# jermp/dint

Hardware: AMD Instinct MI355X
Metric: M ints/sec decoded (vroom single_packed_dint) (higher is better)
Workload: dtype u32

## Files before the change

dint_amd/csrc/hip/dint_kernels.hpp:

```cpp
#pragma once
#include <hip/hip_runtime.h>
#include <stdint.h>

#include "dint_hip.h"

namespace dint_dev {

#ifndef DINT_STORE_AUX
#define DINT_STORE_AUX 2
#endif
#ifndef DINT_BLOCK_THREADS
#define DINT_BLOCK_THREADS 1024
#endif
#ifndef DINT_FF_OPEN
#define DINT_FF_OPEN 4
#endif
#ifndef DINT_MAX_STRAGGLERS
#define DINT_MAX_STRAGGLERS 4096
#endif
#ifndef DINT_SLOT_BURST
#define DINT_SLOT_BURST 2
#endif
static_assert(DINT_SLOT_BURST == 1 || DINT_SLOT_BURST == 2, "DINT_SLOT_BURST: 1 or 2");
#ifndef DINT_SLOT_GLOBAL
#define DINT_SLOT_GLOBAL (DINT_SLOT_BURST == 2)
#endif
#ifndef DINT_SLOT_LATE
#define DINT_SLOT_LATE 0
#endif
#ifndef DINT_GATHER_AUX
#define DINT_GATHER_AUX 0
#endif

constexpr uint32_t kWave = 64;
constexpr uint32_t kBlockThreads = DINT_BLOCK_THREADS;
constexpr uint32_t kWavesPerBlock = kBlockThreads / kWave;
constexpr uint32_t kBlocksPerCU = 1;
constexpr uint32_t kLdsWords = 160 * 1024 / 4;
constexpr uint32_t kSPL = 4;
constexpr uint32_t kTileSlots = kWave * kSPL;
#ifndef DINT_GROUPS
#define DINT_GROUPS 2
#endif
constexpr uint32_t kGroups = DINT_GROUPS;
constexpr uint32_t kRounds = 8 / kGroups;
constexpr uint32_t kMaxCap = 2048;
constexpr uint32_t kFwWords = 2 * 64 + 4;
constexpr uint32_t kDeltaWords = kTileSlots + 4;
#ifndef DINT_STAGE_CELLS
#define DINT_STAGE_CELLS 176
#endif
constexpr uint32_t kStageWords = 4 * DINT_STAGE_CELLS;
#ifdef DINT_PROFILE
constexpr uint32_t kProfWords = 16;
#else
constexpr uint32_t kProfWords = 0;
#endif
constexpr uint32_t kScratchWords = kFwWords + kDeltaWords + kStageWords + kProfWords;
constexpr uint32_t kClassTableWords = 328 + 24;
constexpr uint32_t kDescWordAt = 328;
constexpr uint32_t kHotImageWords = kLdsWords - kClassTableWords - kWavesPerBlock * kScratchWords;
constexpr uint32_t kZeroHalves = 256;
constexpr uint32_t kMetaCold = 1u << 23;
constexpr uint32_t kMetaSlow = 1u << 22;
constexpr uint32_t kMetaOffMask = (1u << 20) - 2;
constexpr uint32_t kMetaPacked8 = 1u;
constexpr uint32_t kMetaException = 1u << 20;
constexpr uint32_t kQueueShards = 8;
constexpr uint32_t kQueueStride = 32;
constexpr uint32_t kChunkShards = 32;
constexpr uint32_t kChunkCounterLineAt = 1;
constexpr uint32_t kQueueLines = kQueueShards + 1 + kChunkShards;
constexpr uint32_t kClockWordAt = 16;
constexpr uint32_t kChunkDryWordAt = 24;
constexpr uint32_t kUnitDryWordAt = 25;
constexpr uint32_t kMaxUnitInts = 1u << 28;

#include "kernels/wave_basics.inc"
#include "kernels/tile.inc"
#include "kernels/segment.inc"
#include "kernels/bundles.inc"

}
#include "dint_query_kernels.hpp"
namespace dint_dev {

#include "kernels/index.inc"
#include "kernels/kernel_body.inc"
#include "kernels/query_pages.inc"

__global__ void debug_wave_scan_kernel(const uint32_t* in, uint32_t* out) {
    out[threadIdx.x] = wave_inclusive_sum(in[threadIdx.x]);
}

}
```

dint_amd/csrc/hip/kernels/bundles.inc:

```
__device__ __forceinline__ void decode_unit_single(const decode_args& a, const wave_ctx& c, uint64_t unit_index, prof_t& pf) {
    const dint_unit* up = a.units + unit_index;
    const uint64_t out_off = up->out_off;
    const uint32_t n = up->n;
    if (n == 0 || n > kMaxUnitInts || out_off > a.out_capacity || a.out_capacity - out_off < n || (a.only_full && n != 256)) return;
    const uint64_t in_off = uniform64(up->in_off);
    chain_io ch{};
    volatile uint8_t* const flag = a.unit_base ? a.gaps_left + unit_index : nullptr;
    if (flag && c.lane == 0) *flag = 0;
    const uint64_t end = decode_segment<16, kRounds, kGroups, 0>(a, c, a.dict.first, in_off, n, a.out + out_off, ch, pf, false, false,
                                                                 a.unit_base ? a.unit_base + unit_index : nullptr,
                                                                 a.unit_base ? a.gaps_left + unit_index : nullptr);
    if (a.end_off && c.lane == 0) a.end_off[unit_index] = end;
    if (flag && n <= 256) {
        uint32_t left = 0;
        if (c.lane == 0) left = *flag, *flag = 0;
        if (uniform(left) != 0) gaps_to_docids_here(a.out + out_off, n, uniform(a.unit_base[unit_index]), c.lane);
    }
}

constexpr uint32_t kBundleMaxInts = 256;
constexpr uint32_t kBundleMaxBytes = 504;

constexpr uint32_t kChunkUnits = 64;
__global__ __launch_bounds__(256) void bundle_schedule_kernel(const dint_unit* units, const uint32_t* spans, uint64_t n_units,
                                                              const uint8_t* enc, uint64_t enc_bytes, uint64_t out_capacity,
                                                              uint32_t only_full, uint32_t multi, uint32_t chunked, uint8_t* sched,
                                                              uint32_t* block_items, u32x4* urec, uint64_t* cbase) {
    __shared__ uint32_t lanes[256], pre[256];
    __shared__ uint32_t place[256];
    __shared__ uint8_t start[256];
    const uint32_t tid = threadIdx.x;
    const uint64_t i = uint64_t(blockIdx.x) * 256 + tid;
    uint32_t L = 0, sel = 0;
    uint64_t in = 0, out = 0;
    uint32_t n = 0;
    if (i < n_units) {
        in = units[i].in_off;
        out = units[i].out_off;
        n = units[i].n;
    }
    const uint64_t in0 = (uint64_t(uint32_t(__shfl(uint32_t(in >> 32), 0))) << 32) | uint32_t(__shfl(uint32_t(in), 0));
    const uint64_t out0 = (uint64_t(uint32_t(__shfl(uint32_t(out >> 32), 0))) << 32) | uint32_t(__shfl(uint32_t(out), 0));
    if (i < n_units) {
        const uint64_t nxt = spans ? in + spans[i] : (i + 1 < n_units ? units[i + 1].in_off : enc_bytes);
        if (n >= 1 && n <= kBundleMaxInts && (!only_full || n == 256) && nxt > in && nxt - in <= kBundleMaxBytes &&
            nxt <= enc_bytes && out <= out_capacity && out_capacity - out >= n && in >= in0 && nxt - in0 + 16 <= 0xFFFFFFFFull && out >= out0 &&
            out - out0 < (chunked ? (1ull << 28) : (1ull << 32))) {
            if (!multi) {
                const uint32_t l = uint32_t((nxt - in + 7) >> 3);
                if (l <= kWave - 1 && in + 8ull * l <= enc_bytes) L = l;
            } else {
                sel = enc[in];
                const uint32_t stride = sel >= 6 ? 4u : 8u;
                const uint32_t l = uint32_t((nxt - in - 1 + stride - 1) / stride);
                if (sel < 12 && l >= 1 && l <= kWave - 1 && in + 1 + uint64_t(stride) * l + 8 <= enc_bytes) L = l;
            }
        }
    }
    lanes[tid] = L | (n << 8);
    pre[tid] = (L != 0 && tid != 0 && i < n_units && out == units[i - 1].out_off + units[i - 1].n) ? 1u : 0u;
    __syncthreads();
    if (chunked) {
        start[tid] = L != 0 ? 0 : 1;
        place[tid] = 0;
    } else if ((tid & 63u) == 0) {
        uint32_t in_use = 0, ints = 0, prev_l = 0;
#pragma unroll 16
        for (uint32_t j = tid; j != tid + 64; ++j) {
            const uint32_t l = lanes[j] & 255u, m = lanes[j] >> 8;
            const bool cont = l != 0 && prev_l != 0 && pre[j] != 0 && in_use + l <= kWave && ints + m <= kMaxCap;
            start[j] = cont ? 0 : 1;
            in_use = cont ? in_use + l : l;
            ints = cont ? ints + m : m;
            prev_l = l;
        }
    }
    __syncthreads();
    uint32_t c = 0;
    if (start[tid] != 0 && i < n_units) {
        c = 1;
        if (L != 0 && !chunked)
            while (tid + c < 256 && ((tid + c) & 63u) != 0 && i + c < n_units && !start[tid + c]) ++c;
    }
    const bool alone = c == 1 && (L == 0 || !chunked) && !(chunked && only_full && n != 256);
    const bool item = alone || (!chunked && c > 1);
    const int n_items = __syncthreads_count(item);
    if (tid == 0) block_items[blockIdx.x] = uint32_t(n_items);
    if (i >= n_units) return;
    sched[i] = uint8_t(item ? c : 0);
    u32x4 r;
    r.x = uint32_t(in - in0);
    r.y = uint32_t(out - out0);
    r.z = ((n - 1u) & 255u) | (L << 8) | (sel << 14) | (c << 18);
    r.w = chunked ? place[tid] : 0u;
    urec[i] = r;
    if ((tid & 63u) == 0) {
        cbase[2 * (i >> 6)] = in0;
        cbase[2 * (i >> 6) + 1] = out0;
    }
}

__global__ __launch_bounds__(64) void bundle_pack_kernel(u32x4* urec, uint64_t n_units) {
    __shared__ uint32_t zs[64][65];
    constexpr uint32_t kOpen = DINT_FF_OPEN;
    const uint32_t tid = threadIdx.x;
    const uint64_t base = (uint64_t(blockIdx.x) * 64 + tid) * kChunkUnits;
    for (uint32_t j = 0; j != kChunkUnits; ++j) zs[tid][j] = base + j < n_units ? urec[base + j].z : 0u;
    uint32_t used[kOpen], mem[kOpen], id[kOpen], n_open = 0, next_id = 0;
#pragma unroll
    for (uint32_t k = 0; k != kOpen; ++k) used[k] = 0, mem[k] = 0, id[k] = 0;
    for (uint32_t j = 0; j != kChunkUnits; ++j) {
        const uint32_t z = zs[tid][j];
        const uint32_t l = (z >> 8) & 63u;
        uint32_t b = kOpen;
#pragma unroll
        for (uint32_t k = 0; k != kOpen; ++k)
            if (b == kOpen && k < n_open && used[k] + l <= kWave && mem[k] < 8) b = k;
        const bool fresh = b == kOpen;
        if (fresh) {
            b = n_open < kOpen ? n_open : 0u;
            if (n_open == kOpen) {
                uint32_t most = used[0];
#pragma unroll
                for (uint32_t k = 1; k != kOpen; ++k)
                    if (used[k] > most) most = used[k], b = k;
            }
        }
        uint32_t pl = 0;
#pragma unroll
        for (uint32_t k = 0; k != kOpen; ++k)
            if (k == b && l != 0) {
                if (fresh) id[k] = next_id, used[k] = 0, mem[k] = 0;
                pl = id[k] | (used[k] << 8) | (mem[k] << 16) | (mem[k] == 0 ? 1u << 31 : 0u);
                used[k] += l;
                mem[k] += 1;
            }
        if (fresh && l != 0) {
            next_id += 1;
            n_open += n_open < kOpen ? 1u : 0u;
        }
        zs[tid][j] = pl;
    }
    for (uint32_t j = 0; j != kChunkUnits; ++j) {
        const uint32_t pl = zs[tid][j];
        if (base + j < n_units && pl != 0) {
            u32x4 r = urec[base + j];
            r.z = (r.z & ~(127u << 18)) | ((pl >> 31) << 18);
            r.w = pl & 0x7FFFFFFFu;
            urec[base + j] = r;
        }
    }
}

__global__ __launch_bounds__(256) void split_units_kernel(const uint32_t* items, uint32_t n_items, const dint_unit* units, const uint8_t* enc,
                                                          uint64_t enc_bytes, uint64_t out_capacity, dict_view dv, u32x4* urec, uint64_t* cbase,
                                                          uint32_t* left_items, uint32_t* n_left) {
    const uint32_t j = blockIdx.x * 256 + threadIdx.x;
    if (j >= n_items) return;
    const dint_unit u = units[items[j]];
    const dint_unit u0 = units[items[j & ~31u]];
    const uint64_t in0 = u0.in_off, out0 = u0.out_off;
    if ((j & 31u) == 0) {
// ... 786 lines not shown
```

dint_amd/csrc/hip/kernels/kernel_body.inc:

```
struct query_pages {
    const dint_block_ref* blocks;
    const uint32_t* ids;
    const uint32_t* count;
    uint64_t bound;
    uint32_t retire;
    const uint32_t* page_query;
    const uint32_t* term_first;
    const uint32_t* term_blocks;
    const uint32_t* block_max;
    uint32_t* target;
    uint32_t* needed;
    uint32_t* rank;
    uint32_t* touched;
    uint32_t* n_touched;
    uint32_t hash_mask;
};
template <bool MULTI>
__device__ __forceinline__ void decode_query_page(const decode_args& a, const wave_ctx& c, const query_pages& qp, uint64_t page, prof_t& pf);

template <bool ALL = true>
__device__ __forceinline__ decode_args own_scalars(const decode_args& k) {
    decode_args a = k;
    asm volatile("" : "+s"(a.dict.tables), "+s"(a.dict.lds_image), "+s"(a.dict.descs), "+s"(a.dict.tables_bytes),
                 "+s"(a.dict.heads_base), "+s"(a.dict.tails_base), "+s"(a.dict.goff_base), "+s"(a.dict.gtable_base), "+s"(a.dict.hot_words),
                 "+s"(a.dict.first.meta_base), "+s"(a.dict.first.hot_base), "+s"(a.dict.first.hot_k));
    asm volatile("" : "+s"(a.enc), "+s"(a.enc_bytes), "+s"(a.units), "+s"(a.n_units), "+s"(a.out),
                 "+s"(a.out_capacity), "+s"(a.end_off), "+s"(a.queue), "+s"(a.n_shards), "+s"(a.only_full));
    if (ALL) asm volatile("" : "+s"(a.sched), "+s"(a.items), "+s"(a.item_cnt), "+s"(a.n_items), "+s"(a.urec), "+s"(a.cbase), "+s"(a.chunk_queue), "+s"(a.spans),
                 "+s"(a.plus_one), "+s"(a.unit_base), "+s"(a.gaps_left));
    return a;
}

template <bool MULTI, bool INDEX, bool QUERY = false, bool BUNDLES_ONLY = false>
__device__ __forceinline__ void decode_kernel_body(const decode_args& kernarg, const query_pages* qp = nullptr,
                                                   const round_tail* tail = nullptr, const tails_args* short_blocks = nullptr,
                                                   uint32_t karg_at = 0) {
    decode_args a_ = own_scalars<(MULTI || INDEX || QUERY)>(kernarg);
    if (!INDEX) {
        a_.unit_base = nullptr;
        a_.gaps_left = nullptr;
        a_.plus_one = 0;
        a_.only_full = 0;
    }
    const decode_args a = a_;
    const uint64_t clock0 = __builtin_amdgcn_s_memtime();
    extern __shared__ __attribute__((aligned(16))) uint32_t lds[];
    uint64_t q_work = 0;
    if (QUERY) {
        q_work = qp->bound;
        if (qp->count) q_work = uniform(*qp->count) < q_work ? uniform(*qp->count) : q_work;
    }
    const bool q_idle = QUERY && uint64_t(blockIdx.x) * kWavesPerBlock >= q_work;
    if (!q_idle) {
    if (!QUERY) {
        for (uint32_t i = threadIdx.x; 4 * i < a.dict.hot_words; i += kBlockThreads)
            reinterpret_cast<u32x4*>(lds)[i] = reinterpret_cast<const u32x4*>(a.dict.lds_image)[i];
    } else {
        constexpr uint32_t kSteps = (kHotImageWords / 4 + kBlockThreads - 1) / kBlockThreads;
        u32x4 part[kSteps];
#pragma unroll
        for (uint32_t k = 0; k != kSteps; ++k) {
            const uint32_t i = threadIdx.x + k * kBlockThreads;
            if (4 * i < a.dict.hot_words) part[k] = reinterpret_cast<const u32x4*>(a.dict.lds_image)[i];
        }
#pragma unroll
        for (uint32_t k = 0; k != kSteps; ++k) {
            const uint32_t i = threadIdx.x + k * kBlockThreads;
            if (4 * i < a.dict.hot_words) reinterpret_cast<u32x4*>(lds)[i] = part[k];
        }
    }
    uint16_t* const cls = reinterpret_cast<uint16_t*>(lds + a.dict.hot_words);
    build_class_table(cls);
    uint32_t* const descs = lds + a.dict.hot_words + kDescWordAt;
    if (threadIdx.x < 24) descs[threadIdx.x] = MULTI ? reinterpret_cast<const uint32_t*>(a.dict.descs)[threadIdx.x] : 0u;
    const uint32_t lane = lane_id();
    const uint32_t wave = uniform(threadIdx.x / kWave);
    uint32_t* const scratch = lds + a.dict.hot_words + kClassTableWords + wave * kScratchWords;
    for (uint32_t i = lane; i < kFwWords; i += kWave) scratch[i] = 0;
    __syncthreads();
    wave_ctx c;
    c.lds = lds;
    c.cls = cls;
    c.descs = descs;
    c.scratch = scratch;
    c.lane = lane;
    c.rs_dict = __builtin_amdgcn_make_buffer_rsrc(const_cast<uint8_t*>(a.dict.tables), 0, int(a.dict.tables_bytes), 0x00020000);
    c.heads_base = a.dict.heads_base;
    c.tails_base = a.dict.tails_base;
    c.goff_base = a.dict.goff_base;
    c.gtable_base = a.dict.gtable_base;
    const uint32_t shard = blockIdx.x % a.n_shards;
    const uint64_t n_work = QUERY ? q_work : a.sched ? uint64_t(uniform(*a.n_items)) : a.n_units;
    const uint64_t per_shard = (n_work + a.n_shards - 1) / a.n_shards;
    uint32_t cur = shard;
    auto ask = [&]() -> uint32_t {
        uint32_t j = 0;
        if (lane == 0) j = __hip_atomic_fetch_add(a.queue + cur * kQueueStride, 1u, __ATOMIC_RELAXED, __HIP_MEMORY_SCOPE_AGENT);
        return j;
    };
    auto take = [&](uint32_t ticket) -> uint64_t {
        uint32_t j = uniform(ticket);
        for (;;) {
            const uint64_t first = per_shard * cur;
            const uint64_t size = first >= n_work ? 0 : (n_work - first < per_shard ? n_work - first : per_shard);
            if (j < size) return first + j;
            const uint32_t next = next_open_counter(a.chunk_queue + kUnitDryWordAt, a.n_shards, cur, lane);
            if (next == ~0u) return ~0ull;
            cur = next;
            j = uniform(ask());
        }
    };
    prof_t pf;
#ifdef DINT_PROFILE
    prof_begin(pf, scratch + kScratchWords - kProfWords, lane);
#endif
    if (INDEX && !QUERY && short_blocks) {
        if (short_blocks->zero_next != nullptr && blockIdx.x == gridDim.x - 1)
            for (uint32_t i = threadIdx.x; i < short_blocks->zero_words; i += kBlockThreads) short_blocks->zero_next[i] = 0;
        SECTION(pf, 5, "short_blocks");
        tails_phase(a.enc, a.enc_bytes, *short_blocks, uint32_t(scratch - lds), lane);
        SECTION(pf, 0, "outside");
    }
    if (QUERY) {
        const uint64_t stride = uint64_t(gridDim.x) * kWavesPerBlock;
        for (uint64_t page = uint64_t(blockIdx.x) * kWavesPerBlock + wave; page < n_work; page += stride) decode_query_page<MULTI>(a, c, *qp, page, pf);
    }
    uint64_t w = BUNDLES_ONLY || QUERY ? ~0ull : take(ask());
    while (!BUNDLES_ONLY && !QUERY && w != ~0ull) {
        SECTION(pf, 14, "draw");
        uint32_t ticket = ask();
        const uint64_t uu = uniform64(!QUERY && a.sched ? uint64_t(a.items[w]) : w);
        if (QUERY) {
            decode_query_page<MULTI>(a, c, *qp, uu, pf);
        } else if (MULTI) {
            decode_unit_multi(a, c, uu, pf);
        } else {
            const uint32_t cc = uniform(a.sched ? uint32_t(a.item_cnt[w]) : 1u);
            if (__builtin_expect(cc > 1, 0)) decode_bundle_listed<false>(a, c, uu, cc, pf);
            else decode_unit_single(a, c, uu, pf);
        }
        asm volatile("" : "+v"(ticket));
        w = take(ticket);
    }
    if ((MULTI || (INDEX && a.only_full)) && !QUERY && a.sched && a.urec) {
        decode_bundle_chunks<MULTI, (MULTI && !INDEX && BUNDLES_ONLY)>(a, c, pf);
    }
#ifdef DINT_PROFILE
    prof_end(pf);
#endif
    }
    if (blockIdx.x == 0 && threadIdx.x == 0 && (a.urec || !a.sched))
    {
#if defined(__HIP_DEVICE_COMPILE__)
        typedef __attribute__((address_space(4))) const uint8_t constant_u8;
        constant_u8* kp = (constant_u8*)__builtin_amdgcn_kernarg_segment_ptr();
        asm volatile("" : "+s"(kp));
        uint64_t* const clk = *(uint64_t* __attribute__((address_space(4))) const*)(kp + karg_at + offsetof(decode_args, clock));
        *clk = __builtin_amdgcn_s_memtime() - clock0;
#else
        (void)clock0, (void)karg_at;
#endif
    }
    if (QUERY) {
        if (!tail->done) return;
        __shared__ uint32_t last;
        if (gridDim.x != 1) __threadfence();
        __syncthreads();
        if (gridDim.x != 1) {
            if (threadIdx.x == 0) last = atomicAdd(tail->done, 1u) == gridDim.x - 1 ? 1u : 0u;
            __syncthreads();
            if (!last) return;
            __threadfence();
        }
        and_round_tail(*tail);
    }
}

#ifndef DINT_MIN_WAVES
#define DINT_MIN_WAVES 1
#endif
__global__ __launch_bounds__(kBlockThreads, DINT_MIN_WAVES) void decode_single_kernel(decode_args a) {
    decode_kernel_body<false, false>(a);
}
__global__ __launch_bounds__(kBlockThreads, DINT_MIN_WAVES) void decode_multi_kernel(decode_args a) {
    decode_kernel_body<true, false>(a);
}
__global__ __launch_bounds__(kBlockThreads, DINT_MIN_WAVES) __attribute__((amdgpu_num_vgpr(126))) void decode_multi_bundles_kernel(decode_args a) {
    decode_kernel_body<true, false, false, true>(a);
}
__global__ __launch_bounds__(kBlockThreads, DINT_MIN_WAVES) void decode_single_index_kernel(decode_args a, tails_args t) {
    decode_kernel_body<false, true>(a, nullptr, nullptr, &t);
}
__global__ __launch_bounds__(kBlockThreads, DINT_MIN_WAVES) void decode_multi_index_kernel(decode_args a, tails_args t) {
    decode_kernel_body<true, true>(a, nullptr, nullptr, &t);
}
__global__ __launch_bounds__(kBlockThreads, DINT_MIN_WAVES) void decode_single_index_bundles_kernel(decode_args a, tails_args t) {
    decode_kernel_body<false, true, false, true>(a, nullptr, nullptr, &t);
}
__global__ __launch_bounds__(kBlockThreads, DINT_MIN_WAVES) void decode_multi_index_bundles_kernel(decode_args a, tails_args t) {
    decode_kernel_body<true, true, false, true>(a, nullptr, nullptr, &t);
}
__global__ __launch_bounds__(kBlockThreads, DINT_MIN_WAVES) void decode_single_index_pair_kernel(decode_args a, decode_args b, tails_args t) {
    decode_kernel_body<false, true, false, true>(a, nullptr, nullptr, &t);
    __syncthreads();
    decode_kernel_body<false, true, false, true>(b, nullptr, nullptr, nullptr, uint32_t(sizeof(decode_args)));
}
__global__ __launch_bounds__(kBlockThreads, DINT_MIN_WAVES) void decode_multi_index_pair_kernel(decode_args a, decode_args b, tails_args t) {
    decode_kernel_body<true, true, false, true>(a, nullptr, nullptr, &t);
    __syncthreads();
    decode_kernel_body<true, true, false, true>(b, nullptr, nullptr, nullptr, uint32_t(sizeof(decode_args)));
}
```

dint_amd/csrc/hip/kernels/segment.inc:

```
template <int W, uint32_t ROUNDS, uint32_t GROUPS, int CHAINED_T>
__device__ __forceinline__ uint64_t decode_segment(const decode_args& a, const wave_ctx& c, const dict_desc& dd, uint64_t in_off,
                                                   uint32_t n, uint32_t* const out, chain_io& ch, prof_t& pf,
                                                   bool narrow_rt = false, bool chained_rt = false,
                                                   const uint32_t* block_base = nullptr, uint8_t* gaps_left = nullptr) {
    SECTION(pf, 11, "segment_prologue");
    docid_bases gb;
    if (block_base != nullptr) gb.v = *block_base;
    const bool narrow = W == 0 ? narrow_rt : W == 8;
    const bool CHAINED = CHAINED_T < 0 ? chained_rt : CHAINED_T != 0;
    const uint32_t kSlotBytes = narrow ? 1u : 2u;
    const uint32_t kTileBytes = kTileSlots * kSlotBytes;
    const uint16_t* const rows = c.cls + (!narrow ? 0 : kRows16);
    const uint32_t lane = c.lane;
    const uint32_t hot_k = dd.hot_k;
    uint32_t* const out_u = reinterpret_cast<uint32_t*>(uniform64(reinterpret_cast<uint64_t>(out)));
    const __amdgpu_buffer_rsrc_t rs_out = __builtin_amdgcn_make_buffer_rsrc(out_u, 0, int(uniform(n) * 4), 0x00020000);
    uint8_t* const lds_rw = reinterpret_cast<uint8_t*>(const_cast<uint32_t*>(c.lds));
    const uint32_t stage_byte0 = uint32_t(reinterpret_cast<const uint8_t*>(stage_of(c.scratch)) - lds_rw);

    constexpr bool kPaired = DINT_SLOT_BURST == 2 && W == 16 && CHAINED_T == 0;
    constexpr bool kGlobalSlots = DINT_SLOT_GLOBAL != 0 && W == 16 && CHAINED_T == 0;
    constexpr bool kLateSlots = DINT_SLOT_LATE != 0 && W == 16 && CHAINED_T == 0;
    const uint64_t in_off_u = uniform64(in_off);
    uint64_t slot_byte = in_off_u;
    uint32_t room = 0;
    if (kPaired && in_off_u <= a.enc_bytes) room = uniform(a.enc_bytes - in_off_u < 0xFFFFFFFFull ? uint32_t(a.enc_bytes - in_off_u) : 0xFFFFFFFFu);
    tile_regs cur;
    uint64_t nxt_raw;
    meta_regs mr;
    head_regs hr;
    uint64_t raw1, raw2 = 0;
    if (CHAINED) {
        unpack_slots(narrow, chain_tile(narrow, ch.data, 0, lane), cur);
        raw1 = chain_tile(narrow, ch.data, 1, lane);
        slot_byte += kTileBytes;
    } else {
        uint64_t raw0 = load_lane_slots<kGlobalSlots>(narrow, a.enc, slot_byte, lane, a.enc_bytes);
        slot_byte += kTileBytes;
        raw1 = load_lane_slots<kGlobalSlots>(narrow, a.enc, slot_byte, lane, a.enc_bytes);
        slot_byte += kTileBytes;
        raw2 = load_lane_slots<kGlobalSlots>(narrow, a.enc, slot_byte, lane, a.enc_bytes);
        asm volatile("" : "+v"(raw0), "+v"(raw1), "+v"(raw2));
        unpack_slots(narrow, raw0, cur);
    }
    ch.valid = false;
    struct tile_class {
        uint32_t row;
        uint32_t carry_out;
        bool special;
        bool tile_exc;
    };
    auto classify = [&](const tile_regs& tr, uint32_t carry_in) -> tile_class {
        tile_class k{kPlainRow, 0u, false, false};
        uint32_t smin = tr.s[0];
#pragma unroll
        for (uint32_t j = 1; j != kSPL; ++j) smin = smin < tr.s[j] ? smin : tr.s[j];
        k.special = __builtin_expect(__ballot(smin < 2) != 0 || carry_in != 0, 0);
        if (k.special) {
            uint32_t lo = 0;
#pragma unroll
            for (uint32_t j = kSPL; j-- != 0;) lo = 3 * lo + (2u - (tr.s[j] < 2 ? tr.s[j] : 2u));
            uint32_t st_in = lane == 0 ? carry_in : 0u;
            uint32_t row;
            for (;;) {
                row = rows[st_in * 81 + lo];
                uint32_t prev = from_lane_below((row >> 8) & 7u);
                if (lane == 0) prev = carry_in;
                if (__ballot(prev != st_in) == 0) break;
                st_in = prev;
            }
            k.row = row;
            k.carry_out = readlane((row >> 8) & 7u, 63);
            k.tile_exc = __ballot((row & 0xF0u) != 0) != 0;
        }
        return k;
    };
    tile_class kc = classify(cur, 0u);
    request_metas(c, dd.hot_base, hot_k, dd.meta_base, cur, mr, hr, kc.row & 15u);
    asm volatile("" : "+v"(raw1), "+v"(raw2));
    nxt_raw = raw1;

    uint32_t produced = 0;
    uint64_t tile_base = in_off_u;
    uint32_t end_slot = 0;
    MARK("loop_top");

    while (produced < n) {
        uint64_t raw3;
        if (!kPaired && !kLateSlots) {
            slot_byte += kTileBytes;
            raw3 = load_lane_slots<kGlobalSlots>(narrow, a.enc, slot_byte, lane, a.enc_bytes);
        }

        SECTION(pf, 1, "1_classify");
        take_metas(hot_k, mr, hr, cur);
        if (!kPaired && kLateSlots) {
            slot_byte += kTileBytes;
            raw3 = load_lane_slots<kGlobalSlots>(narrow, a.enc, slot_byte, lane, a.enc_bytes);
        }
        if (kPaired) {
            if (uint32_t(slot_byte - tile_base) == kTileBytes) {
                const uint64_t pair_byte = slot_byte + kTileBytes;
                slot_byte += 2 * kTileBytes;
                if (uint32_t(slot_byte - in_off_u) + kTileBytes <= room) {
                    raw2 = load_lane_slots<kGlobalSlots, true>(narrow, a.enc, pair_byte, lane, a.enc_bytes);
                    raw3 = load_lane_slots<kGlobalSlots, true>(narrow, a.enc, slot_byte, lane, a.enc_bytes);
                } else {
                    raw2 = load_lane_slots<kGlobalSlots>(narrow, a.enc, pair_byte, lane, a.enc_bytes);
                    raw3 = load_lane_slots<kGlobalSlots>(narrow, a.enc, slot_byte, lane, a.enc_bytes);
                }
            } else {
                asm volatile("" : "=v"(raw3));
            }
        }
        const bool special = kc.special;
        const uint32_t row = kc.row;
        const uint32_t carry_out = kc.carry_out;
        const bool tile_exc = kc.tile_exc;

        SECTION(pf, 2, "2_sizes");
        tile_slots t;
        uint32_t lv1[kSPL] = {1u, 1u, 1u, 1u};
        if (special) {
#pragma unroll
            for (uint32_t k = 0; k != kSPL; ++k) {
                cur.m[k] &= uint32_t(__builtin_amdgcn_sbfe(~row, k, 1));
                lv1[k] = __builtin_amdgcn_ubfe(~row, k, 1);
            }
        }
        const bool tile_slow_dict = __ballot(((cur.m[0] | cur.m[1] | cur.m[2] | cur.m[3]) & kMetaSlow) != 0) != 0;
        uint32_t e[kSPL];
#pragma unroll
        for (uint32_t k = 0; k != kSPL; ++k) {
            e[k] = cur.m[k] >> 24;
            t.need[k] = __builtin_amdgcn_ubfe(cur.m[k], 20, 2);
            t.src2[k] = cur.m[k] & kMetaOffMask;
        }
        bool wide[kSPL] = {false, false, false, false};
        if (tile_exc) {
            uint32_t w32[kSPL];
            if (!narrow) {
                const uint32_t p01 = (cur.s[1] << 16) | cur.s[0], p23 = (cur.s[3] << 16) | cur.s[2];
                const uint32_t next0 = readlane(uint32_t(nxt_raw), 0);
                uint32_t nlo = from_lane_above(p01);
                if (lane == 63) nlo = next0;
                w32[0] = __builtin_amdgcn_alignbit(p23, p01, 16);
                w32[1] = p23;
                w32[2] = __builtin_amdgcn_alignbit(nlo, p23, 16);
                w32[3] = nlo;
            } else {
                const uint32_t b = cur.s[0] | (cur.s[1] << 8) | (cur.s[2] << 16) | (cur.s[3] << 24);
                const uint32_t next0 = readlane(uint32_t(nxt_raw), 0);
                uint32_t nlo = from_lane_above(b);
                if (lane == 63) nlo = next0;
                w32[0] = __builtin_amdgcn_alignbit(nlo, b, 8);
                w32[1] = __builtin_amdgcn_alignbit(nlo, b, 16);
                w32[2] = __builtin_amdgcn_alignbit(nlo, b, 24);
                w32[3] = nlo;
            }
#pragma unroll
            for (uint32_t k = 0; k != kSPL; ++k) {
                const uint32_t excM = uint32_t(__builtin_amdgcn_sbfe(row, 4 + k, 1));
                const uint32_t lit = w32[k] & ((0u - cur.s[k]) | 0xFFFFu) & excM;
                hr.q[k].y = (hr.q[k].y & ~excM) | lit;
                wide[k] = lit > 0xFFFFu;
            }
        }
        t.off[0] = 0;
        t.off[1] = e[0] + lv1[0];
        t.off[2] = t.off[1] + e[1] + lv1[1];
        t.off[3] = t.off[2] + e[2] + lv1[2];
        t.lsum = t.off[3] + e[3] + lv1[3];
        uint32_t hdrcnt = 4;
        uint32_t pincl;
        if (special) {
            hdrcnt = uint32_t(__builtin_popcount(~row & 15u));
            pincl = wave_inclusive_sum((hdrcnt << 24) | t.lsum);
        } else {
            pincl = wave_inclusive_sum(t.lsum);
        }
        t.obase = (pincl & 0xFFFFFFu) - t.lsum;
        const uint32_t remaining = n - produced;
        t.total = readlane(pincl, 63) & 0xFFFFFFu;
        const bool last_tile = t.total >= remaining;
        const bool plain = !special && !last_tile && t.total <= ROUNDS * GROUPS * 256;
        uint32_t slowb = 0;
        if (!plain) {
            t.row = row;
            t.liveb = ~row & 15u;
            t.rbase = special ? (pincl - ((hdrcnt << 24) | t.lsum)) >> 24 : 4 * lane;
            t.nlive = hdrcnt;
            if (last_tile) {
                t.total = remaining;
                uint32_t cand = 0, lb = 0;
                t.nlive = 0;
#pragma unroll
                for (uint32_t k = 0; k != kSPL; ++k) {
                    const uint32_t pos = t.obase + t.off[k];
                    const bool act = ((t.liveb >> k) & 1u) != 0 && pos < remaining;
                    if (act) {
                        const bool exc = ((row >> (4 + k)) & 1u) != 0;
                        cand = kSPL * lane + k + 1 + (exc ? (!narrow ? cur.s[k] + 1 : 2 * cur.s[k] + 2) : 0u);
                        ++t.nlive;
                        lb |= 1u << k;
                    } else {
                        t.need[k] = 0;
                    }
                }
                t.liveb = lb;
                t.lsum = t.obase < remaining ? (t.obase + t.lsum < remaining ? t.lsum : remaining - t.obase) : 0u;
                const uint64_t am = __ballot(cand != 0);
                end_slot = readlane(cand, 63u - uint32_t(__builtin_clzll(am | 1ull)));
            }
            if (tile_slow_dict) {
#pragma unroll
                for (uint32_t k = 0; k != kSPL; ++k)
                    slowb |= ((cur.m[k] >> 22) & (t.liveb >> k) & ~(row >> (4 + k)) & 1u) << k;
            }
        } else if (tile_slow_dict) {
#pragma unroll
            for (uint32_t k = 0; k != kSPL; ++k) slowb |= ((cur.m[k] >> 22) & 1u) << k;
        }
        uint32_t cell_addr[kSPL];
        const uint32_t cells = allocate_cells(t, stage_byte0, cell_addr);
        if (cells > kStageCells) {
#pragma unroll
            for (uint32_t k = 0; k != kSPL; ++k)
                if (t.need[k] != 0 && cell_addr[k] + 16 * t.need[k] > stage_byte0 + 16 * kStageCells) {
                    t.need[k] = 0;
                    slowb |= 1u << k;
                }
        }
#pragma unroll
        for (uint32_t k = 0; k != kSPL; ++k) t.src2[k] = t.need[k] != 0 ? cell_addr[k] : t.src2[k];
        const bool tile_wide = tile_exc && __ballot(wide[0] || wide[1] || wide[2] || wide[3]) != 0;
        const bool tile_slow = __ballot(slowb != 0) != 0;
        if (CHAINED && last_tile) {
            const uint64_t nb = tile_base + uint64_t(kSlotBytes) * end_slot;
            if (ch.more && nb + 1 + kChainBytes <= a.enc_bytes) chain_request(a.enc, nb, lane, ch);
        }
        SECTION(pf, 8, "8_wait");
        uint64_t raw3w = raw3;
        asm volatile("" : "+v"(raw3w));
        if (kPaired) asm volatile("" : "+v"(raw2));
        if (CHAINED) asm volatile("" : "+v"(ch.sel), "+v"(ch.data.x), "+v"(ch.data.y), "+v"(ch.data.z), "+v"(ch.data.w));
        uint32_t t3[kSPL];
        heads_into_cells<W == 16>(lds_rw, t, hr, wide);
        const bool tile_big = __ballot((t.need[0] | t.need[1] | t.need[2] | t.need[3]) > 1u) != 0;
        if (tile_big) {
#pragma unroll
            for (uint32_t k = 0; k != kSPL; ++k) {
                const uint32_t tail = c.tails_base + 32 * (dd.meta_base + cur.s[k]);
                if (t.need[k] > 1u) hr.q[k] = __builtin_amdgcn_raw_buffer_load_b128(c.rs_dict, tail, 0, 0);
                if (t.need[k] > 2u) t3[k] = __builtin_amdgcn_raw_buffer_load_b32(c.rs_dict, tail + 16, 0, 0);
            }
        }
        const bool as_docids = block_base != nullptr && !tile_slow && produced == 0 && last_tile && t.total <= ROUNDS * GROUPS * 256;
        if (block_base != nullptr && !as_docids && lane == 0) *gaps_left = 1;
        gb.on = as_docids;
        if (block_base != nullptr) asm volatile("" : "+v"(gb.v));
        expand_tile<ROUNDS, GROUPS>(t, plain, tile_wide, a.plus_one, gb, produced, c.lds, c.scratch, rs_out, lane, pf, [&]() {
#pragma unroll
            for (uint32_t k = 0; k != kSPL; ++k) asm volatile("" : "+v"(hr.q[k]), "+v"(t3[k]));
            if (tile_big) {
#pragma unroll
                for (uint32_t k = 0; k != kSPL; ++k) {
                    if (t.need[k] > 1u) *reinterpret_cast<u32x4*>(lds_rw + t.src2[k] + 12) = hr.q[k];
                    if (t.need[k] > 2u) *reinterpret_cast<uint32_t*>(lds_rw + t.src2[k] + 28) = t3[k];
                }
            }
            wave_lds_fence();
            SECTION(pf, 3, "3_prefetch");
            if (!last_tile) {
                asm volatile("" : "+v"(nxt_raw));
                tile_regs nxt;
                unpack_slots(narrow, nxt_raw, nxt);
                kc = classify(nxt, carry_out);
                request_metas(c, dd.hot_base, hot_k, dd.meta_base, nxt, mr, hr, kc.row & 15u);
            }
        });

        SECTION(pf, 10, "10_tail");
        if (tile_slow)
            slow_stores(narrow, c, t, slowb, a.plus_one, produced, n, a.enc + tile_base + uint64_t(kSPL * kSlotBytes) * lane, dd.hot_base,
                           hot_k, dd.meta_base, rs_out);
        SECTION(pf, 5, "10_rotate");
        produced += t.total;
        if (produced < n) tile_base += kTileBytes;

        asm volatile("" : "+v"(nxt_raw));
        unpack_slots(narrow, nxt_raw, cur);
        nxt_raw = CHAINED ? raw3w : raw2;
        raw2 = raw3w;
    }
    SECTION(pf, 13, "epilogue");
    return tile_base + uint64_t(kSlotBytes) * end_slot;
}
```

dint_amd/csrc/hip/kernels/tile.inc:

```
struct wave_ctx {
    const uint32_t* lds;
    const uint16_t* cls;
    const uint32_t* descs;
    uint32_t* scratch;
    uint32_t lane;
    __amdgpu_buffer_rsrc_t rs_dict;
    uint32_t heads_base, tails_base, goff_base, gtable_base;
};

__device__ __forceinline__ uint32_t* fw_of(uint32_t* scratch) { return scratch; }
__device__ __forceinline__ uint32_t* delta_of(uint32_t* scratch) { return scratch + kFwWords; }
__device__ __forceinline__ uint32_t* stage_of(uint32_t* scratch) { return scratch + kFwWords + kDeltaWords; }

__device__ __forceinline__ void request_metas(const wave_ctx& c, uint32_t hot_base, uint32_t hot_k, uint32_t meta_base,
                                              const tile_regs& t, meta_regs& mr, head_regs& hr, uint32_t payload = 0) {
#pragma unroll
    for (uint32_t k = 0; k != kSPL; ++k) mr.h[k] = c.lds[hot_base + (t.s[k] < hot_k ? t.s[k] : hot_k)];
#pragma unroll
    for (uint32_t k = 0; k != kSPL; ++k)
        if (t.s[k] >= hot_k && ((payload >> k) & 1u) == 0)
            hr.q[k] = __builtin_amdgcn_raw_buffer_load_b128(c.rs_dict, c.heads_base + 16 * (meta_base + t.s[k]), 0, 0);
}
__device__ __forceinline__ void take_metas(uint32_t hot_k, meta_regs& mr, head_regs& hr, tile_regs& t) {
#pragma unroll
    for (uint32_t k = 0; k != kSPL; ++k) asm volatile("" : "+v"(hr.q[k]));
    asm volatile("" : "+v"(mr.h[0]), "+v"(mr.h[1]), "+v"(mr.h[2]), "+v"(mr.h[3]));
#pragma unroll
    for (uint32_t k = 0; k != kSPL; ++k) t.m[k] = t.s[k] < hot_k ? mr.h[k] : hr.q[k].x;
}


constexpr uint32_t kChainBytes = 16 * kWave;
struct chain_io {
    u32x4 data;
    uint32_t sel;
    bool more;
    bool valid;
};

__device__ __forceinline__ void chain_request(const uint8_t* enc, uint64_t selector_byte, uint32_t lane, chain_io& ch) {
    ch.sel = enc[selector_byte];
    ch.data = reinterpret_cast<const u32x4_a1*>(enc + selector_byte + 1 + 16u * lane)->v;
    ch.valid = true;
}

__device__ __forceinline__ uint64_t chain_tile(bool narrow, const u32x4& d, uint32_t t, uint32_t lane) {
    if (!narrow) {
        const int src = int(32 * t + (lane >> 1));
        const uint32_t x = __shfl(d.x, src), y = __shfl(d.y, src), z = __shfl(d.z, src), w = __shfl(d.w, src);
        const bool hi = (lane & 1u) != 0;
        return (uint64_t(hi ? w : y) << 32) | (hi ? z : x);
    }
    const int src = int(16 * t + (lane >> 2));
    const uint32_t x = __shfl(d.x, src), y = __shfl(d.y, src), z = __shfl(d.z, src), w = __shfl(d.w, src);
    const uint32_t c = lane & 3u;
    return c == 0 ? x : c == 1 ? y : c == 2 ? z : w;
}

struct tile_slots {
    uint32_t off[kSPL];
    uint32_t src2[kSPL];
    uint32_t need[kSPL];
    uint32_t lsum, obase;
    uint32_t total;
    uint32_t row;
    uint32_t liveb;
    uint32_t rbase, nlive;
    __device__ __forceinline__ uint32_t lord(uint32_t k) const {
        return k == 0 ? 0u : k == 1 ? (row >> 11) & 1u : k == 2 ? (row >> 12) & 3u : (row >> 14) & 3u;
    }
};
constexpr uint32_t kPlainRow = (1u << 11) | (2u << 12) | (3u << 14);
constexpr uint32_t kStageCells = kStageWords / 4;

__device__ __forceinline__ uint32_t allocate_cells(const tile_slots& t, uint32_t stage_byte0, uint32_t (&cell_addr)[kSPL]) {
    const uint32_t pre1 = t.need[0], pre2 = pre1 + t.need[1], pre3 = pre2 + t.need[2], mine = pre3 + t.need[3];
    const uint32_t incl = wave_inclusive_sum(mine);
    cell_addr[0] = stage_byte0 + 16 * (incl - mine);
    cell_addr[1] = cell_addr[0] + 16 * pre1;
    cell_addr[2] = cell_addr[0] + 16 * pre2;
    cell_addr[3] = cell_addr[0] + 16 * pre3;
    return readlane(incl, 63);
}

template <bool PACKED8>
__device__ __forceinline__ void heads_into_cells(uint8_t* lds_rw, tile_slots& t, head_regs& hr, const bool (&wide)[kSPL]) {
#pragma unroll
    for (uint32_t k = 0; k != kSPL; ++k)
        if (t.need[k] != 0) {
            if (PACKED8 && t.need[k] == 2u && (hr.q[k].x & kMetaPacked8) != 0) {
                u32x4& q = hr.q[k];
                *reinterpret_cast<uint32_t*>(lds_rw + t.src2[k] + 16) = __builtin_amdgcn_perm(0u, q.z, 0x0c030c02u);
                q.w = __builtin_amdgcn_perm(0u, q.z, 0x0c010c00u);
                q.z = __builtin_amdgcn_perm(0u, q.y, 0x0c030c02u);
                q.y = __builtin_amdgcn_perm(0u, q.y, 0x0c010c00u);
                t.need[k] = 1;
            }
            *reinterpret_cast<u32x4*>(lds_rw + t.src2[k]) = hr.q[k];
            t.src2[k] += 4u + (wide[k] ? 1u : 0u);
        }
}

constexpr uint32_t kDeltaBias = 4096;
__device__ __forceinline__ uint32_t delta_word(uint32_t src2, uint32_t rel) {
    return __builtin_rotateright32(src2, 1) - rel + kDeltaBias;
}

__device__ __forceinline__ void rank_bases(uint8_t* fw, uint32_t lane) {
    const uint32_t flags = *reinterpret_cast<const uint32_t*>(fw + 8 * lane);
    const uint32_t cnt = uint32_t(__builtin_popcount(flags));
    *reinterpret_cast<uint32_t*>(fw + 8 * lane + 4) = wave_inclusive_sum(cnt) - cnt - 1u;
}

__device__ __forceinline__ void tables_plain(const tile_slots& t, uint8_t* fw, uint8_t* delta, uint32_t lane) {
    uint32_t rel[kSPL];
    rel[0] = t.obase;
#pragma unroll
    for (uint32_t k = 1; k != kSPL; ++k) rel[k] = t.obase + t.off[k];
    u32x4 d;
#pragma unroll
    for (uint32_t k = 0; k != kSPL; ++k) {
        uint32_t* const fword = reinterpret_cast<uint32_t*>(fw + ((rel[k] >> 2) & 0x1F8u));
        __hip_atomic_fetch_or(fword, 1u << (rel[k] & 31u), __ATOMIC_RELAXED, __HIP_MEMORY_SCOPE_WAVEFRONT);
        d[k] = delta_word(t.src2[k], rel[k]);
    }
    *reinterpret_cast<u32x4*>(delta + 16 * lane) = d;
    rank_bases(fw, lane);
}

__device__ __forceinline__ void tables_general(const tile_slots& t, uint8_t* fw, uint8_t* delta, bool inb, uint32_t done,
                                               uint32_t rdone, uint32_t lane) {
    const uint32_t inbM = inb ? ~0u : 0u;
    const uint32_t rel0 = t.obase - done, ord0 = t.rbase - rdone;
#pragma unroll
    for (uint32_t k = 0; k != kSPL; ++k) {
        const uint32_t lv = uint32_t(__builtin_amdgcn_sbfe(t.liveb, k, 1)) & inbM;
        const uint32_t rel = rel0 + t.off[k];
        uint32_t* const fword = reinterpret_cast<uint32_t*>(fw + ((rel >> 2) & 0x1F8u));
        __hip_atomic_fetch_or(fword, lv & (1u << (rel & 31u)), __ATOMIC_RELAXED, __HIP_MEMORY_SCOPE_WAVEFRONT);
        const uint32_t ord = (lv & (ord0 + t.lord(k))) | (~lv & (kTileSlots + k));
        *reinterpret_cast<uint32_t*>(delta + 4 * ord) = delta_word(t.src2[k], rel);
    }
    rank_bases(fw, lane);
}

struct group_out {
    uint32_t* base;
    uint32_t unit_n, rel_out;
};
struct docid_bases {
    bool on = false;
    uint32_t v = 0;
};

__device__ __forceinline__ void gaps_to_docids_here(uint32_t* out, uint32_t n, uint32_t base, uint32_t lane) {
    __builtin_amdgcn_s_waitcnt(0x0F70);
    uint32_t g[4], local = 0;
#pragma unroll
    for (uint32_t k = 0; k != 4; ++k) {
        const uint32_t i = 4 * lane + k;
        g[k] = i < n ? __hip_atomic_load(out + i, __ATOMIC_RELAXED, __HIP_MEMORY_SCOPE_AGENT) + 1u : 0u;
        local += g[k];
    }
    uint32_t run = base + wave_inclusive_sum(local) - local - 1u;
#pragma unroll
    for (uint32_t k = 0; k != 4; ++k) {
        const uint32_t i = 4 * lane + k;
        run += g[k];
        if (i < n) out[i] = run;
    }
}

template <uint32_t ROUNDS, uint32_t GROUPS>
__device__ __forceinline__ void expand_batch(uint32_t bt, uint32_t out_int, const uint8_t* lds_bytes, const uint8_t* fw,
                                             const uint8_t* delta, const __amdgpu_buffer_rsrc_t rs_out, uint32_t lane,
                                             uint32_t plus_one, const docid_bases& gb, const group_out* go = nullptr) {
    const uint32_t sh = (4 * lane) & 31u;
    const uint32_t pair_byte = (lane >> 3) * 8;
    const uint32_t posb = 4 * lane - kDeltaBias;
    out_int = uniform(out_int);
#pragma unroll
// ... 140 lines not shown
```

Before: 818,800.

## Keep paired slot prefetch in reserved VGPRs with manual vmcnt waits

Adds a windowed slot prefetch mode for the single-unit decode path. Paired tile-slot loads are issued as inline-asm buffer loads into hard-coded registers v124-v127, outside compiler tracking, and head loads become untracked buffer loads. Both are ordered with explicit s_waitcnt vmcnt waits, so a pending pair load can stay in flight across a tile iteration instead of being waited on by compiler-inserted waits. The kernel's VGPR budget is capped at 62 so the allocator stays clear of the reserved registers. This relies on fragile register assumptions and manual wait counts, and the VGPR cap may force spills.

After: 826,800, median of 6. No clear change (+1.0%).

```diff
diff --git a/dint_amd/csrc/hip/dint_kernels.hpp b/dint_amd/csrc/hip/dint_kernels.hpp
--- a/dint_amd/csrc/hip/dint_kernels.hpp
+++ b/dint_amd/csrc/hip/dint_kernels.hpp
@@ -27,6 +27,9 @@
 #endif
 #ifndef DINT_SLOT_LATE
 #define DINT_SLOT_LATE 0
+#endif
+#ifndef DINT_SLOT_WINDOW
+#define DINT_SLOT_WINDOW 1
 #endif
 #ifndef DINT_GATHER_AUX
 #define DINT_GATHER_AUX 0
diff --git a/dint_amd/csrc/hip/kernels/bundles.inc b/dint_amd/csrc/hip/kernels/bundles.inc
--- a/dint_amd/csrc/hip/kernels/bundles.inc
+++ b/dint_amd/csrc/hip/kernels/bundles.inc
@@ -1,3 +1,4 @@
+template <int WINDOW>
 __device__ __forceinline__ void decode_unit_single(const decode_args& a, const wave_ctx& c, uint64_t unit_index, prof_t& pf) {
     const dint_unit* up = a.units + unit_index;
     const uint64_t out_off = up->out_off;
@@ -7,7 +8,7 @@
     chain_io ch{};
     volatile uint8_t* const flag = a.unit_base ? a.gaps_left + unit_index : nullptr;
     if (flag && c.lane == 0) *flag = 0;
-    const uint64_t end = decode_segment<16, kRounds, kGroups, 0>(a, c, a.dict.first, in_off, n, a.out + out_off, ch, pf, false, false,
+    const uint64_t end = decode_segment<16, kRounds, kGroups, 0, WINDOW>(a, c, a.dict.first, in_off, n, a.out + out_off, ch, pf, false, false,
                                                                  a.unit_base ? a.unit_base + unit_index : nullptr,
                                                                  a.unit_base ? a.gaps_left + unit_index : nullptr);
     if (a.end_off && c.lane == 0) a.end_off[unit_index] = end;
diff --git a/dint_amd/csrc/hip/kernels/kernel_body.inc b/dint_amd/csrc/hip/kernels/kernel_body.inc
--- a/dint_amd/csrc/hip/kernels/kernel_body.inc
+++ b/dint_amd/csrc/hip/kernels/kernel_body.inc
@@ -137,7 +137,7 @@
         } else {
             const uint32_t cc = uniform(a.sched ? uint32_t(a.item_cnt[w]) : 1u);
             if (__builtin_expect(cc > 1, 0)) decode_bundle_listed<false>(a, c, uu, cc, pf);
-            else decode_unit_single(a, c, uu, pf);
+            else decode_unit_single<(INDEX ? 0 : 1)>(a, c, uu, pf);
         }
         asm volatile("" : "+v"(ticket));
         w = take(ticket);
@@ -179,7 +179,12 @@
 #ifndef DINT_MIN_WAVES
 #define DINT_MIN_WAVES 1
 #endif
-__global__ __launch_bounds__(kBlockThreads, DINT_MIN_WAVES) void decode_single_kernel(decode_args a) {
+#if DINT_SLOT_WINDOW
+#define DINT_SINGLE_VGPRS __attribute__((amdgpu_num_vgpr(62)))
+#else
+#define DINT_SINGLE_VGPRS
+#endif
+__global__ __launch_bounds__(kBlockThreads, DINT_MIN_WAVES) DINT_SINGLE_VGPRS void decode_single_kernel(decode_args a) {
     decode_kernel_body<false, false>(a);
 }
 __global__ __launch_bounds__(kBlockThreads, DINT_MIN_WAVES) void decode_multi_kernel(decode_args a) {
diff --git a/dint_amd/csrc/hip/kernels/segment.inc b/dint_amd/csrc/hip/kernels/segment.inc
--- a/dint_amd/csrc/hip/kernels/segment.inc
+++ b/dint_amd/csrc/hip/kernels/segment.inc
@@ -1,4 +1,4 @@
-template <int W, uint32_t ROUNDS, uint32_t GROUPS, int CHAINED_T>
+template <int W, uint32_t ROUNDS, uint32_t GROUPS, int CHAINED_T, int WINDOW = 0>
 __device__ __forceinline__ uint64_t decode_segment(const decode_args& a, const wave_ctx& c, const dict_desc& dd, uint64_t in_off,
                                                    uint32_t n, uint32_t* const out, chain_io& ch, prof_t& pf,
                                                    bool narrow_rt = false, bool chained_rt = false,
@@ -21,10 +21,13 @@
     constexpr bool kPaired = DINT_SLOT_BURST == 2 && W == 16 && CHAINED_T == 0;
     constexpr bool kGlobalSlots = DINT_SLOT_GLOBAL != 0 && W == 16 && CHAINED_T == 0;
     constexpr bool kLateSlots = DINT_SLOT_LATE != 0 && W == 16 && CHAINED_T == 0;
+    constexpr bool kWindow = kPaired && DINT_SLOT_WINDOW != 0 && WINDOW != 0;
     const uint64_t in_off_u = uniform64(in_off);
     uint64_t slot_byte = in_off_u;
     uint32_t room = 0;
     if (kPaired && in_off_u <= a.enc_bytes) room = uniform(a.enc_bytes - in_off_u < 0xFFFFFFFFull ? uint32_t(a.enc_bytes - in_off_u) : 0xFFFFFFFFu);
+    const __amdgpu_buffer_rsrc_t rs_enc = __builtin_amdgcn_make_buffer_rsrc(const_cast<uint8_t*>(a.enc) + in_off_u, 0, int(room), 0x00020000);
+    bool pair_behind = false;
     tile_regs cur;
     uint64_t nxt_raw;
     meta_regs mr;
@@ -76,9 +79,10 @@
         return k;
     };
     tile_class kc = classify(cur, 0u);
-    request_metas(c, dd.hot_base, hot_k, dd.meta_base, cur, mr, hr, kc.row & 15u);
+    request_metas<kWindow>(c, dd.hot_base, hot_k, dd.meta_base, cur, mr, hr, kc.row & 15u);
     asm volatile("" : "+v"(raw1), "+v"(raw2));
     nxt_raw = raw1;
+    if (kWindow) pair_put_second(raw2);
 
     uint32_t produced = 0;
     uint64_t tile_base = in_off_u;
@@ -93,12 +97,13 @@
         }
 
         SECTION(pf, 1, "1_classify");
+        if (kWindow) wait_heads(uniform(pair_behind ? 1u : 0u) != 0);
         take_metas(hot_k, mr, hr, cur);
         if (!kPaired && kLateSlots) {
             slot_byte += kTileBytes;
             raw3 = load_lane_slots<kGlobalSlots>(narrow, a.enc, slot_byte, lane, a.enc_bytes);
         }
-        if (kPaired) {
+        if (kPaired && !kWindow) {
             if (uint32_t(slot_byte - tile_base) == kTileBytes) {
                 const uint64_t pair_byte = slot_byte + kTileBytes;
                 slot_byte += 2 * kTileBytes;
@@ -240,9 +245,12 @@
             if (ch.more && nb + 1 + kChainBytes <= a.enc_bytes) chain_request(a.enc, nb, lane, ch);
         }
         SECTION(pf, 8, "8_wait");
-        uint64_t raw3w = raw3;
-        asm volatile("" : "+v"(raw3w));
-        if (kPaired) asm volatile("" : "+v"(raw2));
+        uint64_t raw3w = 0;
+        if (!kWindow) {
+            raw3w = raw3;
+            asm volatile("" : "+v"(raw3w));
+        }
+        if (kPaired && !kWindow) asm volatile("" : "+v"(raw2));
         if (CHAINED) asm volatile("" : "+v"(ch.sel), "+v"(ch.data.x), "+v"(ch.data.y), "+v"(ch.data.z), "+v"(ch.data.w));
         uint32_t t3[kSPL];
         heads_into_cells<W == 16>(lds_rw, t, hr, wide);
@@ -260,6 +268,7 @@
         gb.on = as_docids;
         if (block_base != nullptr) asm volatile("" : "+v"(gb.v));
         expand_tile<ROUNDS, GROUPS>(t, plain, tile_wide, a.plus_one, gb, produced, c.lds, c.scratch, rs_out, lane, pf, [&]() {
+            if (kWindow) wait_heads(false);
 #pragma unroll
             for (uint32_t k = 0; k != kSPL; ++k) asm volatile("" : "+v"(hr.q[k]), "+v"(t3[k]));
             if (tile_big) {
@@ -276,7 +285,12 @@
                 tile_regs nxt;
                 unpack_slots(narrow, nxt_raw, nxt);
                 kc = classify(nxt, carry_out);
-                request_metas(c, dd.hot_base, hot_k, dd.meta_base, nxt, mr, hr, kc.row & 15u);
+                request_metas<kWindow>(c, dd.hot_base, hot_k, dd.meta_base, nxt, mr, hr, kc.row & 15u);
+                if (kWindow && t.total > ROUNDS * GROUPS * 256) {
+                    wait_heads(false);
+#pragma unroll
+                    for (uint32_t k = 0; k != kSPL; ++k) asm volatile("" : "+v"(hr.q[k]));
+                }
             }
         });
 
@@ -290,8 +304,30 @@
 
         asm volatile("" : "+v"(nxt_raw));
         unpack_slots(narrow, nxt_raw, cur);
-        nxt_raw = CHAINED ? raw3w : raw2;
-        raw2 = raw3w;
+        if (!kWindow) {
+            nxt_raw = CHAINED ? raw3w : raw2;
+            raw2 = raw3w;
+        } else {
+            const uint32_t req_rel = uniform(uint32_t(slot_byte - in_off_u));
+            const bool more = uniform(produced < n ? 1u : 0u) != 0;
+            pair_behind = false;
+            if (req_rel - uniform(uint32_t(tile_base - in_off_u)) != kTileBytes) {
+                nxt_raw = pair_take_first();
+            } else {
+                nxt_raw = pair_take_second();
+                if (more) {
+                    const uint64_t pair_byte = slot_byte + kTileBytes;
+                    slot_byte += 2 * kTileBytes;
+                    if (req_rel + 3 * kTileBytes <= room) {
+                        pair_request(rs_enc, 8 * lane, req_rel + kTileBytes, req_rel + 2 * kTileBytes);
+                        pair_behind = true;
+                    } else {
+                        pair_put_first(load_lane_slots<kGlobalSlots>(narrow, a.enc, pair_byte, lane, a.enc_bytes));
+                        pair_put_second(load_lane_slots<kGlobalSlots>(narrow, a.enc, slot_byte, lane, a.enc_bytes));
+                    }
+                }
+            }
+        }
     }
     SECTION(pf, 13, "epilogue");
     return tile_base + uint64_t(kSlotBytes) * end_slot;
diff --git a/dint_amd/csrc/hip/kernels/tile.inc b/dint_amd/csrc/hip/kernels/tile.inc
--- a/dint_amd/csrc/hip/kernels/tile.inc
+++ b/dint_amd/csrc/hip/kernels/tile.inc
@@ -12,14 +12,29 @@
 __device__ __forceinline__ uint32_t* delta_of(uint32_t* scratch) { return scratch + kFwWords; }
 __device__ __forceinline__ uint32_t* stage_of(uint32_t* scratch) { return scratch + kFwWords + kDeltaWords; }
 
+template <bool UNTRACKED = false>
 __device__ __forceinline__ void request_metas(const wave_ctx& c, uint32_t hot_base, uint32_t hot_k, uint32_t meta_base,
                                               const tile_regs& t, meta_regs& mr, head_regs& hr, uint32_t payload = 0) {
 #pragma unroll
     for (uint32_t k = 0; k != kSPL; ++k) mr.h[k] = c.lds[hot_base + (t.s[k] < hot_k ? t.s[k] : hot_k)];
 #pragma unroll
     for (uint32_t k = 0; k != kSPL; ++k)
-        if (t.s[k] >= hot_k && ((payload >> k) & 1u) == 0)
-            hr.q[k] = __builtin_amdgcn_raw_buffer_load_b128(c.rs_dict, c.heads_base + 16 * (meta_base + t.s[k]), 0, 0);
+        if (t.s[k] >= hot_k && ((payload >> k) & 1u) == 0) {
+            const uint32_t at = c.heads_base + 16 * (meta_base + t.s[k]);
+#if defined(__HIP_DEVICE_COMPILE__)
+            if (UNTRACKED) asm volatile("buffer_load_dwordx4 %0, %1, %2, 0 offen" : "+v"(hr.q[k]) : "v"(at), "s"(c.rs_dict) : "memory");
+            else
+#endif
+                hr.q[k] = __builtin_amdgcn_raw_buffer_load_b128(c.rs_dict, at, 0, 0);
+        }
+}
+__device__ __forceinline__ void wait_heads(bool pair_behind) {
+#if defined(__HIP_DEVICE_COMPILE__)
+    if (pair_behind) asm volatile("s_waitcnt vmcnt(2)" : : : "memory");
+    else asm volatile("s_waitcnt vmcnt(0)" : : : "memory");
+#else
+    (void)pair_behind;
+#endif
 }
 __device__ __forceinline__ void take_metas(uint32_t hot_k, meta_regs& mr, head_regs& hr, tile_regs& t) {
 #pragma unroll
@@ -27,6 +42,43 @@
     asm volatile("" : "+v"(mr.h[0]), "+v"(mr.h[1]), "+v"(mr.h[2]), "+v"(mr.h[3]));
 #pragma unroll
     for (uint32_t k = 0; k != kSPL; ++k) t.m[k] = t.s[k] < hot_k ? mr.h[k] : hr.q[k].x;
+}
+
+__device__ __forceinline__ void pair_request(const __amdgpu_buffer_rsrc_t rs, uint32_t lane_byte, uint32_t first, uint32_t second) {
+#if defined(__HIP_DEVICE_COMPILE__)
+    asm volatile("buffer_load_dwordx2 v[124:125], %0, %1, %2 offen\n\tbuffer_load_dwordx2 v[126:127], %0, %1, %3 offen"
+                 : : "v"(lane_byte), "s"(rs), "s"(first), "s"(second) : "memory", "v124", "v125", "v126", "v127");
+#else
+    (void)rs, (void)lane_byte, (void)first, (void)second;
+#endif
+}
+__device__ __forceinline__ uint64_t pair_take_first() {
+    uint32_t lo = 0, hi = 0;
+#if defined(__HIP_DEVICE_COMPILE__)
+    asm volatile("v_mov_b32 %0, v124\n\tv_mov_b32 %1, v125" : "=v"(lo), "=v"(hi));
+#endif
+    return (uint64_t(hi) << 32) | lo;
+}
+__device__ __forceinline__ uint64_t pair_take_second() {
+    uint32_t lo = 0, hi = 0;
+#if defined(__HIP_DEVICE_COMPILE__)
+    asm volatile("v_mov_b32 %0, v126\n\tv_mov_b32 %1, v127" : "=v"(lo), "=v"(hi));
+#endif
+    return (uint64_t(hi) << 32) | lo;
+}
+__device__ __forceinline__ void pair_put_first(uint64_t raw) {
+#if defined(__HIP_DEVICE_COMPILE__)
+    asm volatile("v_mov_b32 v124, %0\n\tv_mov_b32 v125, %1" : : "v"(uint32_t(raw)), "v"(uint32_t(raw >> 32)) : "v124", "v125");
+#else
+    (void)raw;
+#endif
+}
+__device__ __forceinline__ void pair_put_second(uint64_t raw) {
+#if defined(__HIP_DEVICE_COMPILE__)
+    asm volatile("v_mov_b32 v126, %0\n\tv_mov_b32 v127, %1" : : "v"(uint32_t(raw)), "v"(uint32_t(raw >> 32)) : "v126", "v127");
+#else
+    (void)raw;
+#endif
 }
 
 
```
